# Snoworday/instance-segmentation-attention

Measured on AMD Instinct MI355X. Metric: images/sec @256x256 bs=16 per GPU, higher is better.
Workload: dtype bf16; 1 GPU; train.py step fwd+bwd+update 256x256 bs=16/GPU (bf16); global_batch=16, parallelism=dp1, launch=hipGraph replay

## Files before the change

### instance-segmentation-attention_amd/csrc/conv_fused_bwd.hip

```cpp
#include "common.hpp"
#include "tr_lds.hpp"

int wgrad_slab_reduce_launch(float* ws, float* dw, float* dbias, int gx, int tn, int tk, int N, int cin, int taps,
                             isa_slab_arena* sa, hipStream_t s);

namespace {

struct PwParams {
    const bf16_t *g, *y, *x; bf16_t* dx; const float* w; float* dw;
    int N, K, ldg, ldy, ldx, lddx; long M;
    const float *ysc, *ysh, *ymu, *yis, *yred; float ycnt_inv; int yact; float *ydgamma, *ydbeta;
    const float *xsc, *xsh, *xmu, *xis; int xact; float* xred;
    int accumulate; float* ws;
    const bf16_t* addend; int lda;
    int G;
};

template <int TN, int TK, int YACT, int XMODE>
__global__ __launch_bounds__(256) __attribute__((amdgpu_waves_per_eu(2, 2))) void pw_bn_bwd_kernel(PwParams p) {
    extern __shared__ __attribute__((aligned(16))) char ldsb[];
    constexpr int PMB = 32;
    constexpr int SN = TrStride<TN * 32>::bytes, SK = TrStride<TK * 32>::bytes;
    constexpr int SLAB = PMB * (SN + SK);
    constexpr int VN = TN * 4, VK = TK * 4;
    constexpr int LOADS_N = PMB * VN / 64, LOADS_K = PMB * VK / 64;
    constexpr int RPN = 64 / VN, RPK = 64 / VK;
    constexpr int XACT = XMODE == 1 ? ISA_ACT_RELU6 : (XMODE == 0 ? ISA_ACT_NONE : ACT_RT);
    constexpr int NS = TN * 2;
    const int tid = threadIdx.x, wave = tid >> 6, lane = tid & 63;
    const int r = lane & 31, hh = lane >> 5;
    char* sD = ldsb + wave * SLAB;
    char* sX = sD + PMB * SN;
    const GroupSel gs = group_sel(p.G);
    if (gs.g) {
        const long gm = (long)gs.g * p.M;
        p.g += gm * p.ldg; p.y += gm * p.ldy; p.x += gm * p.ldx; p.dx += gm * p.lddx;
        if (p.addend) p.addend += gm * p.lda;
        p.ysc += gs.g * p.N; p.ysh += gs.g * p.N; p.ymu += gs.g * p.N; p.yis += gs.g * p.N; p.yred += gs.g * ISA_STAT_R * 2 * p.N;
        p.xsc = goff(p.xsc, (long)gs.g * p.K); p.xsh = goff(p.xsh, (long)gs.g * p.K); p.xmu = goff(p.xmu, (long)gs.g * p.K);
        p.xis = goff(p.xis, (long)gs.g * p.K); p.xred = goff(p.xred, (long)gs.g * ISA_STAT_R * 2 * p.K);
    }
    const bool want_xred = XMODE == 1 || (XMODE == 2 && p.xred != nullptr);

    const int cgn = lane % VN, rown = lane / VN, cgk = lane % VK, rowk = lane / VK;
    const int cn0 = cgn * 8, ck0 = cgk * 8;
    const bool nok = cn0 < p.N, kok = ck0 < p.K;
    float* cst = reinterpret_cast<float*>(ldsb + 4 * SLAB);
    float* wl = reinterpret_cast<float*>(ldsb);
    for (int i = tid; i < p.N * p.K; i += 256) wl[i] = p.w[i];
    if (tid < 64) {
        const int cn = min(tid, p.N - 1), ck = min(tid, p.K - 1);
        cst[0 * 64 + tid] = p.ysc[cn]; cst[1 * 64 + tid] = p.ysh[cn]; cst[2 * 64 + tid] = p.ymu[cn];
        float r0 = 0.f, r1 = 0.f;
#pragma unroll
        for (int r = 0; r < ISA_STAT_R; ++r) { r0 += p.yred[r * 2 * p.N + cn]; r1 += p.yred[r * 2 * p.N + p.N + cn]; }
        cst[3 * 64 + tid] = p.yis[cn] * (r1 * p.ycnt_inv);
        cst[4 * 64 + tid] = r0 * p.ycnt_inv;
        if (gs.bx == 0 && tid < p.N) {
            if (p.ydgamma) atomicAdd(p.ydgamma + tid, r1);
            if (p.ydbeta) atomicAdd(p.ydbeta + tid, r0);
        }
        cst[5 * 64 + tid] = (XMODE && p.xsc) ? p.xsc[ck] : 1.f; cst[6 * 64 + tid] = (XMODE && p.xsh) ? p.xsh[ck] : 0.f;
        cst[7 * 64 + tid] = (XMODE && p.xmu) ? p.xmu[ck] : 0.f; cst[8 * 64 + tid] = (XMODE && p.xis) ? p.xis[ck] : 1.f;
    }
    __syncthreads();
    auto ldc = [&](int which, int c0, float (&v)[8]) {
        const f32x4 a = *reinterpret_cast<const f32x4*>(cst + which * 64 + c0), b = *reinterpret_cast<const f32x4*>(cst + which * 64 + c0 + 4);
#pragma unroll
        for (int j = 0; j < 4; ++j) { v[j] = a[j]; v[4 + j] = b[j]; }
    };
    bf16x8 wb[NS][TK];
#pragma unroll
    for (int s = 0; s < NS; ++s)
#pragma unroll
        for (int j = 0; j < TK; ++j)
#pragma unroll
            for (int jj = 0; jj < 8; ++jj) {
                const int n = 16 * s + 8 * hh + jj, k = 32 * j + r;
                wb[s][j][jj] = (bf16_t)((n < p.N && k < p.K) ? wl[n * p.K + k] : 0.f);
            }
    __syncthreads();

    f32x16 acc[TN][TK];
#pragma unroll
    for (int i = 0; i < TN; ++i)
#pragma unroll
        for (int j = 0; j < TK; ++j) acc[i][j] = f32x16{0};
    float s0[8], s1[8];
#pragma unroll
    for (int j = 0; j < 8; ++j) { s0[j] = 0.f; s1[j] = 0.f; }

    bf16x8 rg[LOADS_N], ry[LOADS_N], rx[LOADS_K], rxc[LOADS_K];
    const long nchunks = (p.M + PMB - 1) / PMB;
    auto fetch = [&](long chunk) {
        const long mbase = chunk * PMB;
#pragma unroll
        for (int v = 0; v < LOADS_N; ++v) {
            const long m = mbase + v * RPN + rown;
            rg[v] = bf16x8{0}; ry[v] = bf16x8{0};
            if (m < p.M && nok) {
                rg[v] = *reinterpret_cast<const bf16x8*>(p.g + m * p.ldg + cn0);
                ry[v] = *reinterpret_cast<const bf16x8*>(p.y + m * p.ldy + cn0);
            }
        }
#pragma unroll
        for (int v = 0; v < LOADS_K; ++v) {
            const long m = mbase + v * RPK + rowk;
            rx[v] = bf16x8{0};
            if (m < p.M && kok) rx[v] = *reinterpret_cast<const bf16x8*>(p.x + m * p.ldx + ck0);
        }
    };
    auto stash = [&](long chunk) {
        const long mbase = chunk * PMB;
        {
        float ysc[8], ysh[8], ymu[8], yq[8], yk0[8];
        ldc(0, cn0, ysc); ldc(1, cn0, ysh); ldc(2, cn0, ymu); ldc(3, cn0, yq); ldc(4, cn0, yk0);
#pragma unroll
        for (int v = 0; v < LOADS_N; ++v) {
            const bool ok = (mbase + v * RPN + rown) < p.M && nok;
            bf16x8 o;
#pragma unroll
            for (int j = 0; j < 8; ++j) {
                const float yy = (float)ry[v][j];
                const float dz = (float)rg[v][j] * act_grad_t<YACT>(fmaf(yy, ysc[j], ysh[j]), p.yact);
                const float val = ysc[j] * (dz - yk0[j] - (yy - ymu[j]) * yq[j]);
                o[j] = (bf16_t)((ok && cn0 + j < p.N) ? val : 0.f);
            }
            *reinterpret_cast<bf16x8*>(sD + (v * RPN + rown) * SN + cgn * 16) = o;
        }
        }
        float xsc[8], xsh[8];
        ldc(5, ck0, xsc); ldc(6, ck0, xsh);
#pragma unroll
        for (int v = 0; v < LOADS_K; ++v) {
            const bool ok = (mbase + v * RPK + rowk) < p.M && kok;
            bf16x8 o;
#pragma unroll
            for (int j = 0; j < 8; ++j) {
                const float xr = (float)rx[v][j];
                const float z = XMODE ? act_t<XACT>(fmaf(xr, xsc[j], xsh[j]), p.xact) : xr;
                o[j] = (bf16_t)((ok && ck0 + j < p.K) ? z : 0.f);
            }
            *reinterpret_cast<bf16x8*>(sX + (v * RPK + rowk) * SK + cgk * 16) = o;
            rxc[v] = rx[v];
        }
    };

    const long stride = (long)gs.nbx * 4;
    long chunk = (long)gs.bx * 4 + wave;
    if (chunk < nchunks) fetch(chunk);
    for (; chunk < nchunks; chunk += stride) {
        stash(chunk);
        __builtin_amdgcn_fence(__ATOMIC_RELEASE, "wavefront");
        __builtin_amdgcn_wave_barrier();
        if (chunk + stride < nchunks) fetch(chunk + stride);
        constexpr bool EPI_PREFETCH = TK == 1;
        bf16x8 repi_old[EPI_PREFETCH ? LOADS_K : 1], repi_add[EPI_PREFETCH ? LOADS_K : 1];
        if constexpr (EPI_PREFETCH) {
            const long mb = chunk * PMB;
#pragma unroll
            for (int v = 0; v < LOADS_K; ++v) {
                const long m = mb + v * RPK + rowk;
                repi_old[v] = bf16x8{0}; repi_add[v] = bf16x8{0};
                if (m < p.M && kok) {
                    if (p.accumulate) repi_old[v] = *reinterpret_cast<const bf16x8*>(p.dx + m * p.lddx + ck0);
                    if (p.addend) repi_add[v] = *reinterpret_cast<const bf16x8*>(p.addend + m * p.lda + ck0);
                }
            }
        }
#pragma unroll
        for (int s = 0; s < PMB / 16; ++s) {
            bf16x8 a[TN], b[TK];
#pragma unroll
            for (int i = 0; i < TN; ++i) a[i] = tr_frag(sD, SN, 16 * s, i * 32, lane);
#pragma unroll
            for (int j = 0; j < TK; ++j) b[j] = tr_frag(sX, SK, 16 * s, j * 32, lane);
#pragma unroll
            for (int i = 0; i < TN; ++i)
#pragma unroll
                for (int j = 0; j < TK; ++j)
                    acc[i][j] = __builtin_amdgcn_mfma_f32_32x32x16_bf16(a[i], b[j], acc[i][j], 0, 0, 0);
        }
        f32x16 dxa[TK];
#pragma unroll
        for (int j = 0; j < TK; ++j) dxa[j] = f32x16{0};
#pragma unroll
        for (int s = 0; s < NS; ++s) {
            const bf16x8 a = *reinterpret_cast<const bf16x8*>(sD + r * SN + (16 * s + 8 * hh) * 2);
#pragma unroll
            for (int j = 0; j < TK; ++j)
                dxa[j] = __builtin_amdgcn_mfma_f32_32x32x16_bf16(a, wb[s][j], dxa[j], 0, 0, 0);
        }
        __builtin_amdgcn_fence(__ATOMIC_RELEASE, "wavefront");
        __builtin_amdgcn_wave_barrier();
#pragma unroll
        for (int j = 0; j < TK; ++j)
#pragma unroll
            for (int e = 0; e < 16; ++e) {
                const int row = (e & 3) + 8 * (e >> 2) + 4 * hh;
                *reinterpret_cast<bf16_t*>(sX + row * SK + (32 * j + r) * 2) = (bf16_t)dxa[j][e];
            }
        __builtin_amdgcn_fence(__ATOMIC_RELEASE, "wavefront");
        __builtin_amdgcn_wave_barrier();
        const long mbase = chunk * PMB;
        float xsc[8], xsh[8], xmu[8], xis[8];
        if (want_xred) { ldc(5, ck0, xsc); ldc(6, ck0, xsh); ldc(7, ck0, xmu); ldc(8, ck0, xis); }
#pragma unroll
        for (int v = 0; v < LOADS_K; ++v) {
            const long m = mbase + v * RPK + rowk;
            if (m < p.M && kok) {
                bf16x8 o = *reinterpret_cast<const bf16x8*>(sX + (v * RPK + rowk) * SK + cgk * 16);
                bf16_t* dst = p.dx + m * p.lddx + ck0;
                if (p.accumulate) {
                    bf16x8 old;
                    if constexpr (EPI_PREFETCH) old = repi_old[v]; else old = *reinterpret_cast<const bf16x8*>(dst);
#pragma unroll
                    for (int j = 0; j < 8; ++j) o[j] = (bf16_t)((float)o[j] + (float)old[j]);
                }
                if (p.addend) {
                    bf16x8 ad;
                    if constexpr (EPI_PREFETCH) ad = repi_add[v]; else ad = *reinterpret_cast<const bf16x8*>(p.addend + m * p.lda + ck0);
#pragma unroll
                    for (int j = 0; j < 8; ++j) o[j] = (bf16_t)((float)o[j] + (float)ad[j]);
                }
                *reinterpret_cast<bf16x8*>(dst) = o;
                if (want_xred) {
#pragma unroll
                    for (int j = 0; j < 8; ++j) {
                        const float xr = (float)rxc[v][j];
                        const float dz = (float)o[j] * act_grad_t<XACT>(fmaf(xr, xsc[j], xsh[j]), p.xact);
                        s0[j] += dz; s1[j] += dz * ((xr - xmu[j]) * xis[j]);
                    }
                }
            }
        }
        __builtin_amdgcn_fence(__ATOMIC_RELEASE, "wavefront");
        __builtin_amdgcn_wave_barrier();
    }

    __syncthreads();
    float* red = reinterpret_cast<float*>(ldsb);
    constexpr int ACC_FLOATS = TN * TK * 16 * 64;
    for (int w = 0; w < 4; ++w) {
        if (wave == w) {
#pragma unroll
            for (int i = 0; i < TN; ++i)
#pragma unroll
                for (int j = 0; j < TK; ++j)
#pragma unroll
                    for (int e = 0; e < 16; ++e) {
                        float* q = red + ((i * TK + j) * 16 + e) * 64 + lane;
                        *q = (w == 0 ? 0.f : *q) + acc[i][j][e];
                    }
        }
        __syncthreads();
    }
    constexpr int SLABF = TN * TK * 1024 + TN * 32;
    float* slab = p.ws + (long)blockIdx.x * SLABF;
    if (wave == 0) {
#pragma unroll
        for (int e = 0; e < TN * TK * 16; ++e) slab[e * 64 + lane] = red[e * 64 + lane];
        for (int i = lane; i < TN * 32; i += 64) slab[TN * TK * 1024 + i] = 0.f;
    }
    if (want_xred) {
        __syncthreads();
        float* xr = red;
        for (int i = tid; i < 2 * TK * 32; i += 256) xr[i] = 0.f;
        __syncthreads();
#pragma unroll
        for (int j = 0; j < 8; ++j) {
            const float v0 = row_fold<VK>(s0[j]), v1 = row_fold<VK>(s1[j]);
            if ((lane & 15) < VK) { atomicAdd(&xr[ck0 + j], v0); atomicAdd(&xr[TK * 32 + ck0 + j], v1); }
        }
        __syncthreads();
        for (int i = tid; i < 2 * TK * 32; i += 256) {
            const int which = i / (TK * 32), c = i - which * TK * 32;
            if (c < p.K && xr[i] != 0.f)
                atomicAdd(p.xred + (blockIdx.x & (ISA_STAT_R - 1)) * 2 * p.K + which * p.K + c, xr[i]);
        }
    }
}

template <int TN, int TK, int YACT, int XMODE>
int launch_inst(PwParams& p, long ws_floats, isa_slab_arena* sa, const isa_pro* xfin, int xfin_groups, hipStream_t s) {
    constexpr int SN = TrStride<TN * 32>::bytes, SK = TrStride<TK * 32>::bytes;
    constexpr size_t slab = (size_t)32 * (SN + SK) * 4 + 9 * 64 * 4;
    constexpr size_t redb = ((size_t)TN * TK * 16 * 64 + TN * 32) * 4;
    constexpr size_t lds = slab > redb ? slab : redb;
    const long nchunks = (p.M + 31) / 32;
    const long slabf = (long)TN * TK * 1024 + TN * 32;
    long gx = (nchunks + 3) / 4 * p.G;
    if (gx > 256 * 2) gx = 256 * 2;
    if (int rc = defer_ws(sa, &p.ws, &ws_floats)) return rc;
    const long ws_cap = ws_floats / slabf;
    if (ws_cap < p.G) return sa ? ISA_ENOMEM : ISA_EINVAL;
    if (gx > ws_cap) gx = ws_cap;
    gx = group_grid(gx, p.G);
    if (int rc = fin_standalone(xfin, p.K, xfin_groups, s)) return rc;
    hipLaunchKernelGGL((pw_bn_bwd_kernel<TN, TK, YACT, XMODE>), dim3((unsigned)gx), dim3(256), lds, s, p);
    if (launch_status() != ISA_OK) return ISA_ELAUNCH;
    return wgrad_slab_reduce_launch(p.ws, p.dw, nullptr, (int)gx, TN, TK, p.N, p.K, 1, sa, s);
}

template <int TN, int TK>
int launch_tile(PwParams& p, int xmode, long ws_floats, isa_slab_arena* sa, const isa_pro* xfin, int xfin_groups, hipStream_t s) {
    const bool y6 = p.yact == ISA_ACT_RELU6, y0 = p.yact == ISA_ACT_NONE;
#define PW_X(YA) (xmode == 0 ? launch_inst<TN, TK, YA, 0>(p, ws_floats, sa, xfin, xfin_groups, s) \
                : xmode == 1 ? launch_inst<TN, TK, YA, 1>(p, ws_floats, sa, xfin, xfin_groups, s) \
                             : launch_inst<TN, TK, YA, 2>(p, ws_floats, sa, xfin, xfin_groups, s))
    if (y6) return PW_X(ISA_ACT_RELU6);
    if (y0) return PW_X(ISA_ACT_NONE);
    return PW_X(ACT_RT);
#undef PW_X
}

}

extern "C" int isa_conv1x1_bn_backward(const isa_tensor* g, const isa_tensor* y, const isa_bn_bwd* ybn,
                                       const isa_tensor* x, const isa_pro* xpro, const isa_bn_bwd* xbn,
                                       const float* w, float* dw, const isa_tensor* dx, int32_t accumulate,
                                       const isa_tensor* addend, float* ws, int64_t ws_floats, isa_slab_arena* defer,
                                       void* stream) {
    if (!tensor_ok(g, 8) || !tensor_ok(y, 8) || !tensor_ok(x, 8) || !tensor_ok(dx, 8)) return ISA_EINVAL;
    if (!fin_valid(xpro)) return ISA_EINVAL;
    if (g->dtype != ISA_BF16 || y->dtype != ISA_BF16 || x->dtype != ISA_BF16 || dx->dtype != ISA_BF16) return ISA_EINVAL;
    if (!ybn || !ybn->scale || !ybn->shift || !ybn->mean || !ybn->invstd || !ybn->red || !(ybn->count > 0)) return ISA_EINVAL;
    if (!w || !dw || (!ws && !defer)) return ISA_EINVAL;
    const int N = g->c, K = x->c;
    if (N > 64 || K > 64 || N % 8 || K % 8) return ISA_EINVAL;
    if (y->c != N || dx->c != K) return ISA_EINVAL;
    const isa_tensor* ts[3] = {y, x, dx};
    for (const isa_tensor* t : ts)
        if (t->n != g->n || t->h != g->h || t->w != g->w) return ISA_EINVAL;
    const ProDev xp = make_pro(xpro);
    if (xp.bscale) return ISA_EINVAL;
    if (xbn && (!xbn->mean || !xbn->invstd || !xbn->out_red)) return ISA_EINVAL;
    PwParams p{};
    p.g = (const bf16_t*)g->data; p.y = (const bf16_t*)y->data; p.x = (const bf16_t*)x->data; p.dx = (bf16_t*)dx->data;
    p.w = w; p.dw = dw; p.N = N; p.K = K; p.ldg = g->ld; p.ldy = y->ld; p.ldx = x->ld; p.lddx = dx->ld;
// ... 23 lines not shown
```

### instance-segmentation-attention_amd/csrc/conv_wgrad.hip

```cpp
#include <vector>
#include "common.hpp"
#include "tr_lds.hpp"

int conv3x3_wgrad_tiled_launch(const isa_tensor* x, const isa_tensor* dy, float* dw, float* dbias, float* ws, long ws_floats,
                               isa_slab_arena* sa,
                               hipStream_t s);

namespace {

constexpr int PM = 16;

struct WgParams {
    const void* x; int xh, xw, cin, ldx;
    const void* dy; int dh, dw_, ldd;
    int mh, mw; long M;
    ProDev pro;
    float* dw; float* dbias;
    const int32_t* kmap; int ksrc;
    int N, taps, in_mode, out_mode;
    int groups_k;
    long nchunks;
    long ws_floats;
    int G;
    isa_slab_arena* sa;
// ... 258 lines not shown
        fold_depthwise(d.ws, d.gx, d.gy, d.tk, d.N, d.ksrc, d.dw, d.dbias, lb % d.gy, lb / d.gy, d.rsplit);
    }
}

constexpr long DEFER_MIN_FLOATS = 16L << 20;

static int launch_reduce(const WgParams& p, int gx, int gy, int tn, int tk, hipStream_t s) {
    const int slabf = tn * tk * 1024 + tn * 32;
    const long base_blocks = (long)cdiv(slabf, 256) * gy * p.taps;
    int rsplit = (int)((512 + base_blocks - 1) / base_blocks);
    if (rsplit > 64) rsplit = 64;
    if (rsplit > gx) rsplit = gx;
    if (rsplit < 1) rsplit = 1;
    if (p.sa && p.sa->from_arena) {
        FoldDesc d{p.ws, p.dw, p.dbias, p.kmap, 0, gx, gy, p.taps, p.groups_k, tn, tk, p.N, p.cin, p.ksrc, p.out_mode, 0, 0, 0};
        if (defer_push(p.sa, d, (long)gx * gy * p.taps * slabf)) return ISA_OK;
    }
    WgReduce q{p.ws, p.dw, p.dbias, p.kmap, gx, gy, p.taps, p.groups_k, tn, tk, p.N, p.cin, p.ksrc, p.out_mode, rsplit};
    dim3 grid(cdiv(slabf, 256), gy, p.taps * rsplit);
    hipLaunchKernelGGL(wgrad_reduce_kernel, grid, dim3(256), 0, s, q);
    return launch_status();
}

template <int TN, int TK, int ACT>
__global__ __launch_bounds__(256) void conv_wgrad_bf16_kernel(WgParams p) {
    extern __shared__ __attribute__((aligned(16))) char ldsb[];
    constexpr int PMB = 32;
    constexpr int SN = TrStride<TN * 32>::bytes, SK = TrStride<TK * 32>::bytes;
    constexpr int SLAB = PMB * (SN + SK);
    constexpr int VN = TN * 4, VK = TK * 4;
    constexpr int LOADS_N = PMB * VN / 64, LOADS_K = PMB * VK / 64;
    const int tid = threadIdx.x, wave = tid >> 6, lane = tid & 63;
    const int r = lane & 31, hh = lane >> 5;
    const int gn = blockIdx.y / p.groups_k, gk = blockIdx.y % p.groups_k;
    const int tap = blockIdx.z;
    const int n0 = gn * TN * 32, k0 = gk * TK * 32;
    char* sD = ldsb + wave * SLAB;
    char* sX = sD + PMB * SN;
    const GroupSel gs = group_sel(p.G);
    if (gs.g) {
        p.x = reinterpret_cast<const bf16_t*>(p.x) + (long)gs.g * p.M * p.ldx;
        p.dy = reinterpret_cast<const bf16_t*>(p.dy) + (long)gs.g * p.M * p.ldd;
        p.pro.scale = goff(p.pro.scale, (long)gs.g * p.cin); p.pro.shift = goff(p.pro.shift, (long)gs.g * p.cin);
        p.pro.bscale = goff(p.pro.bscale, (long)gs.g * (p.M / ((long)p.mh * p.mw)) * p.cin);
    }
    const bf16_t* xin = reinterpret_cast<const bf16_t*>(p.x);
    const bf16_t* din = reinterpret_cast<const bf16_t*>(p.dy);
    const bool plain = p.in_mode == ISA_IN_1X1 && p.out_mode == ISA_OUT_PLAIN;

    f32x16 acc[TN][TK];
#pragma unroll
    for (int i = 0; i < TN; ++i)
#pragma unroll
        for (int j = 0; j < TK; ++j) acc[i][j] = f32x16{0};
    float dbs[TN];
#pragma unroll
    for (int i = 0; i < TN; ++i) dbs[i] = 0.f;
    bf16x8 rd[LOADS_N], rx[LOADS_K];
    const long nchunks = (p.M + PMB - 1) / PMB;
    const int cgn = lane % VN, rown = lane / VN, cgk = lane % VK, rowk = lane / VK;
    constexpr int RPN = 64 / VN, RPK = 64 / VK;
    const int cn0 = n0 + cgn * 8, ck0 = k0 + cgk * 8;
    const bool has_aff = p.pro.scale || p.pro.shift;
    const bool has_pro = has_aff || p.pro.bscale || p.pro.act != ISA_ACT_NONE;
    float psc[8], psh[8];
#pragma unroll
    for (int j = 0; j < 8; ++j) {
        const int c = min(ck0 + j, p.cin - 1);
        psc[j] = p.pro.scale ? p.pro.scale[c] : 1.f;
        psh[j] = p.pro.shift ? p.pro.shift[c] : 0.f;
    }

    auto fetch = [&](long chunk) {
        const long mbase = chunk * PMB;
#pragma unroll
        for (int v = 0; v < LOADS_N; ++v) {
            const long m = mbase + v * RPN + rown;
            rd[v] = bf16x8{0};
            if (m < p.M && cn0 < p.N) {
                long row = m;
                if (p.out_mode == ISA_OUT_SHUFFLE2) {
                    const unsigned mu = (unsigned)m, q = mu / (unsigned)p.mw;
                    const int px = (int)(mu - q * (unsigned)p.mw);
                    const unsigned pb = q / (unsigned)p.mh; const int py = (int)(q - pb * (unsigned)p.mh);
                    row = ((long)pb * p.dh + 2 * py + (tap >> 1)) * p.dw_ + 2 * px + (tap & 1);
                }
                const bf16_t* src = din + row * p.ldd + cn0;
                if (cn0 + 8 <= p.N) rd[v] = *reinterpret_cast<const bf16x8*>(src);
                else {
#pragma unroll
                    for (int j = 0; j < 8; ++j) rd[v][j] = (cn0 + j < p.N) ? src[j] : (bf16_t)0.f;
                }
            }
        }
#pragma unroll
        for (int v = 0; v < LOADS_K; ++v) {
            const long m = mbase + v * RPK + rowk;
            rx[v] = bf16x8{0};
            if (m < p.M && ck0 < p.cin) {
                long row = m; bool ok = true; long pb = 0;
                if (!plain || p.pro.bscale) {
                    const unsigned mu = (unsigned)m, q = mu / (unsigned)p.mw;
                    const int px = (int)(mu - q * (unsigned)p.mw);
                    pb = q / (unsigned)p.mh; const int py = (int)(q - (unsigned)pb * (unsigned)p.mh);
                    if (p.in_mode == ISA_IN_3X3) {
                        const int sy = py + tap / 3 - 1, sx = px + tap % 3 - 1;
                        ok = sy >= 0 && sy < p.xh && sx >= 0 && sx < p.xw;
                        row = (pb * p.xh + sy) * p.xw + sx;
                    }
                }
                if (ok) {
                    const bf16_t* src = xin + row * p.ldx + ck0;
                    bf16x8 raw;
                    if (ck0 + 8 <= p.cin) raw = *reinterpret_cast<const bf16x8*>(src);
                    else {
#pragma unroll
                        for (int j = 0; j < 8; ++j) raw[j] = (ck0 + j < p.cin) ? src[j] : (bf16_t)0.f;
                    }
                    if (has_pro) {
                        float z[8];
#pragma unroll
                        for (int j = 0; j < 8; ++j) z[j] = act_t<ACT>(fmaf((float)raw[j], psc[j], psh[j]), p.pro.act);
                        if (p.pro.bscale) {
#pragma unroll
                            for (int j = 0; j < 8; ++j) z[j] *= p.pro.bscale[pb * p.cin + min(ck0 + j, p.cin - 1)];
                        }
                        if (ck0 + 8 > p.cin) {
#pragma unroll
                            for (int j = 0; j < 8; ++j) if (ck0 + j >= p.cin) z[j] = 0.f;
                        }
#pragma unroll
                        for (int j = 0; j < 8; ++j) raw[j] = (bf16_t)z[j];
                    }
                    rx[v] = raw;
                }
            }
        }
    };
    auto stash = [&]() {
#pragma unroll
        for (int v = 0; v < LOADS_N; ++v)
            *reinterpret_cast<bf16x8*>(sD + (v * RPN + rown) * SN + cgn * 16) = rd[v];
#pragma unroll
        for (int v = 0; v < LOADS_K; ++v)
            *reinterpret_cast<bf16x8*>(sX + (v * RPK + rowk) * SK + cgk * 16) = rx[v];
    };

    const long stride = (long)gs.nbx * 4;
    long chunk = (long)gs.bx * 4 + wave;
    if (chunk < nchunks) fetch(chunk);
    for (; chunk < nchunks; chunk += stride) {
        stash();
        __builtin_amdgcn_fence(__ATOMIC_RELEASE, "wavefront");
        __builtin_amdgcn_wave_barrier();
        if (chunk + stride < nchunks) fetch(chunk + stride);
#pragma unroll
        for (int s = 0; s < PMB / 16; ++s) {
            bf16x8 a[TN], b[TK];
#pragma unroll
            for (int i = 0; i < TN; ++i) {
                a[i] = tr_frag(sD, SN, 16 * s, i * 32, lane);
#pragma unroll
                for (int j = 0; j < 8; ++j) dbs[i] += (float)a[i][j];
            }
#pragma unroll
            for (int j = 0; j < TK; ++j) b[j] = tr_frag(sX, SK, 16 * s, j * 32, lane);
#pragma unroll
            for (int i = 0; i < TN; ++i)
#pragma unroll
                for (int j = 0; j < TK; ++j)
                    acc[i][j] = __builtin_amdgcn_mfma_f32_32x32x16_bf16(a[i], b[j], acc[i][j], 0, 0, 0);
        }
        __builtin_amdgcn_fence(__ATOMIC_RELEASE, "wavefront");
        __builtin_amdgcn_wave_barrier();
    }

    __syncthreads();
    float* red = reinterpret_cast<float*>(ldsb);
    constexpr int ACC_FLOATS = TN * TK * 16 * 64;
    for (int w = 0; w < 4; ++w) {
        if (wave == w) {
#pragma unroll
            for (int i = 0; i < TN; ++i)
#pragma unroll
                for (int j = 0; j < TK; ++j)
#pragma unroll
                    for (int e = 0; e < 16; ++e) {
                        float* q = red + ((i * TK + j) * 16 + e) * 64 + lane;
                        *q = (w == 0 ? 0.f : *q) + acc[i][j][e];
                    }
#pragma unroll
            for (int i = 0; i < TN; ++i) {
                const float sv = dbs[i] + __shfl_xor(dbs[i], 32, 64);
                if (hh == 0) { float* q = red + ACC_FLOATS + i * 32 + r; *q = (w == 0 ? 0.f : *q) + sv; }
            }
        }
        __syncthreads();
    }
    if (wave != 0) return;
    constexpr int SLABF = TN * TK * 1024 + TN * 32;
    float* slab = p.ws + (((long)blockIdx.x * gridDim.y + blockIdx.y) * gridDim.z + blockIdx.z) * SLABF;
#pragma unroll
    for (int e = 0; e < TN * TK * 16; ++e) slab[e * 64 + lane] = red[e * 64 + lane];
    for (int i = lane; i < TN * 32; i += 64) slab[TN * TK * 1024 + i] = red[ACC_FLOATS + i];
}

template <int TN, int TK>
int launch_wg_bf16(WgParams& p, int groups_n, const isa_pro* fin, hipStream_t s) {
    constexpr int SN = TrStride<TN * 32>::bytes, SK = TrStride<TK * 32>::bytes;
    const size_t slab = (size_t)32 * (SN + SK) * 4;
    const size_t redb = ((size_t)TN * TK * 16 * 64 + TN * 32) * 4;
    const size_t lds = slab > redb ? slab : redb;
    const int gy = groups_n * p.groups_k;
    const long nchunks = (p.M + 31) / 32;
    const long slabf = (long)TN * TK * 1024 + TN * 32;
    long want = (nchunks + 3) / 4 * p.G;
    long cap = (256L * 2) / ((long)gy * p.taps);
    if (int rc = defer_ws(p.sa, &p.ws, &p.ws_floats)) return rc;
    const long ws_cap = p.ws_floats / (slabf * gy * p.taps);
    if (ws_cap < p.G) return p.sa ? ISA_ENOMEM : ISA_EINVAL;
    if (cap > ws_cap) cap = ws_cap;
    if (cap < 1) cap = 1;
    const int gx = (int)group_grid(want < cap ? want : cap, p.G);
    dim3 grid(gx, gy, p.taps);
    if (int rc = fin_standalone(fin, p.cin, p.G, s)) return rc;
    if (p.pro.act == ISA_ACT_RELU6) hipLaunchKernelGGL((conv_wgrad_bf16_kernel<TN, TK, ISA_ACT_RELU6>), grid, dim3(256), lds, s, p);
    else if (p.pro.act == ISA_ACT_LEAKY && TN == 1 && TK == 1) hipLaunchKernelGGL((conv_wgrad_bf16_kernel<TN, TK, ISA_ACT_LEAKY>), grid, dim3(256), lds, s, p);
    else if (p.pro.act == ISA_ACT_NONE) hipLaunchKernelGGL((conv_wgrad_bf16_kernel<TN, TK, ISA_ACT_NONE>), grid, dim3(256), lds, s, p);
    else hipLaunchKernelGGL((conv_wgrad_bf16_kernel<TN, TK, ACT_RT>), grid, dim3(256), lds, s, p);
    if (launch_status() != ISA_OK) return ISA_ELAUNCH;
    return launch_reduce(p, gx, gy, TN, TK, s);
}


// ... 31 lines not shown
    else { tn = 2; tk = 2; }
    const int groups_n = (nt + tn - 1) / tn;
    p.groups_k = (kt + tk - 1) / tk;
    if constexpr (sizeof(T) == 2) {
        if (tn == 1 && tk == 1) return launch_wg_bf16<1, 1>(p, groups_n, fin, s);
        if (tn == 1 && tk == 2) return launch_wg_bf16<1, 2>(p, groups_n, fin, s);
        if (tn == 2 && tk == 1) return launch_wg_bf16<2, 1>(p, groups_n, fin, s);
        if (tn == 2 && tk == 2) return launch_wg_bf16<2, 2>(p, groups_n, fin, s);
        if (tn == 1 && tk == 4) return launch_wg_bf16<1, 4>(p, groups_n, fin, s);
        if (tn == 4 && tk == 1) return launch_wg_bf16<4, 1>(p, groups_n, fin, s);
        return ISA_EINVAL;
    }
    if (tn == 1 && tk == 1) return launch_wg<T, 1, 1>(p, groups_n, fin, s);
    if (tn == 1 && tk == 2) return launch_wg<T, 1, 2>(p, groups_n, fin, s);
    if (tn == 2 && tk == 1) return launch_wg<T, 2, 1>(p, groups_n, fin, s);
    if (tn == 2 && tk == 2) return launch_wg<T, 2, 2>(p, groups_n, fin, s);
    if (tn == 1 && tk == 4) return launch_wg<T, 1, 4>(p, groups_n, fin, s);
    if (tn == 4 && tk == 1) return launch_wg<T, 4, 1>(p, groups_n, fin, s);
    return ISA_EINVAL;
}

}

extern "C" int isa_conv_wgrad(const isa_tensor* x, const isa_pro* pro, const isa_tensor* dy,
                              float* dw, float* dbias, int32_t in_mode, int32_t out_mode,
                              const int32_t* kmap, int32_t ksrc, float* ws, int64_t ws_floats,
                              isa_slab_arena* defer, void* stream) {
    if (!tensor_ok(x, 8) || !tensor_ok(dy, 8) || !dw || x->dtype != dy->dtype || (!ws && !defer)) return ISA_EINVAL;
    if (!fin_valid(pro)) return ISA_EINVAL;
    if (in_mode == ISA_IN_GATHER2) return ISA_EINVAL;
    WgParams p{};
    p.x = x->data; p.xh = x->h; p.xw = x->w; p.cin = x->c; p.ldx = x->ld;
    p.dy = dy->data; p.dh = dy->h; p.dw_ = dy->w; p.ldd = dy->ld;
    p.mh = x->h; p.mw = x->w; p.M = (long)x->n * x->h * x->w;
    p.pro = make_pro(pro); p.dw = dw; p.dbias = dbias; p.kmap = kmap; p.ksrc = ksrc > 0 ? ksrc : x->c;
    p.in_mode = in_mode; p.out_mode = out_mode; p.ws = ws; p.ws_floats = ws_floats; p.sa = defer;
    if (out_mode == ISA_OUT_SHUFFLE2) {
        if (in_mode != ISA_IN_1X1 || dy->h != 2 * x->h || dy->w != 2 * x->w || dy->n != x->n) return ISA_EINVAL;
        p.taps = 4; p.N = dy->c;
    } else {
        if (dy->h != x->h || dy->w != x->w || dy->n != x->n) return ISA_EINVAL;
        p.taps = in_mode == ISA_IN_3X3 ? 9 : 1; p.N = dy->c;
    }
    p.G = 1;
    const int G = tensor_groups(x);
    if (G > 1 && (p.pro.scale || p.pro.shift)) {
// ... 80 lines not shown
```

### instance-segmentation-attention_amd/csrc/tr_lds.hpp

```cpp
#pragma once
#include "common.hpp"

typedef short s16x4 __attribute__((ext_vector_type(4)));
typedef short s16x8 __attribute__((ext_vector_type(8)));
#define LDS_S16X4(ptr) ((__attribute__((address_space(3))) s16x4*)(ptr))

template <int CH> struct TrStride { static constexpr int bytes = (CH * 2) % 128 == 0 ? CH * 2 + 64 : CH * 2; };

__device__ __forceinline__ bf16x8 tr_frag(const char* tile, int stride_bytes, int pix0, int chan0, int lane) {
    const int g = lane >> 4, i = lane & 15, q = i >> 2, pp = i & 3;
    const char* a = tile + (pix0 + 8 * (g >> 1) + q) * stride_bytes + (chan0 + 16 * (g & 1) + 4 * pp) * 2;
    const s16x4 lo = __builtin_amdgcn_ds_read_tr16_b64_v4i16(LDS_S16X4(a));
    const s16x4 hi = __builtin_amdgcn_ds_read_tr16_b64_v4i16(LDS_S16X4(a + 4 * stride_bytes));
    const s16x8 v = __builtin_shufflevector(lo, hi, 0, 1, 2, 3, 4, 5, 6, 7);
    return __builtin_bit_cast(bf16x8, v);
}
```

Measured before the change: 693.4 images/s.

## Restructure pointwise BN-backward and wgrad kernels: early prefetch, parallel fold, branchless loads

Both backward kernels now issue the first chunk's global loads before the weight and constant setup, so that load latency overlaps with that setup. Guarded loads become branchless loads at clamped addresses, with validity kept as bitmasks or zeroing applied in the stash step. The serialized four-wave LDS accumulation, which needed a block barrier per wave, is replaced by each wave parking its accumulators in its own region and then a parallel 4-way sum on store. In the pointwise kernel the weights are staged as transposed bf16 in LDS so each lane reads them with one vector load. An EPI template flag drops the accumulate/addend epilogue when it is unused, and the x-stat atomics become a slot sum. Optional phase-timing macros are added but compile away by default. The parallel fold uses more LDS, which may reduce occupancy.

```diff
diff --git a/instance-segmentation-attention_amd/csrc/conv_fused_bwd.hip b/instance-segmentation-attention_amd/csrc/conv_fused_bwd.hip
--- a/instance-segmentation-attention_amd/csrc/conv_fused_bwd.hip
+++ b/instance-segmentation-attention_amd/csrc/conv_fused_bwd.hip
@@ -16,9 +16,14 @@
     int G;
 };
 
-template <int TN, int TK, int YACT, int XMODE>
+#ifdef ISA_PHASE_TRACE
+__device__ unsigned long long phase_buf[10];
+#endif
+
+template <int TN, int TK, int YACT, int XMODE, bool EPI>
 __global__ __launch_bounds__(256) __attribute__((amdgpu_waves_per_eu(2, 2))) void pw_bn_bwd_kernel(PwParams p) {
     extern __shared__ __attribute__((aligned(16))) char ldsb[];
+    PHASE_DECL(); PHASE(0);
     constexpr int PMB = 32;
     constexpr int SN = TrStride<TN * 32>::bytes, SK = TrStride<TK * 32>::bytes;
     constexpr int SLAB = PMB * (SN + SK);
@@ -45,9 +50,37 @@
     const int cgn = lane % VN, rown = lane / VN, cgk = lane % VK, rowk = lane / VK;
     const int cn0 = cgn * 8, ck0 = cgk * 8;
     const bool nok = cn0 < p.N, kok = ck0 < p.K;
+    const int cnl = nok ? cn0 : 0, ckl = kok ? ck0 : 0;
+
+    bf16x8 rg[LOADS_N], ry[LOADS_N], rx[LOADS_K], rxc[LOADS_K];
+    const long nchunks = (p.M + PMB - 1) / PMB;
+    auto fetch = [&](long chunk) {
+        const long mbase = chunk * PMB;
+#pragma unroll
+        for (int v = 0; v < LOADS_N; ++v) {
+            const long m = min(mbase + v * RPN + rown, p.M - 1);
+            rg[v] = *reinterpret_cast<const bf16x8*>(p.g + m * p.ldg + cnl);
+            ry[v] = *reinterpret_cast<const bf16x8*>(p.y + m * p.ldy + cnl);
+        }
+#pragma unroll
+        for (int v = 0; v < LOADS_K; ++v) {
+            const long m = min(mbase + v * RPK + rowk, p.M - 1);
+            rx[v] = *reinterpret_cast<const bf16x8*>(p.x + m * p.ldx + ckl);
+        }
+    };
+    const long stride = (long)gs.nbx * 4;
+    long chunk = (long)gs.bx * 4 + wave;
+    if (chunk < nchunks) fetch(chunk);
+
     float* cst = reinterpret_cast<float*>(ldsb + 4 * SLAB);
-    float* wl = reinterpret_cast<float*>(ldsb);
-    for (int i = tid; i < p.N * p.K; i += 256) wl[i] = p.w[i];
+    constexpr int WP = TN * 32 + 8;
+    bf16_t* wl = reinterpret_cast<bf16_t*>(ldsb);
+    float wv[TN * TK * 4];
+#pragma unroll
+    for (int it = 0; it < TN * TK * 4; ++it) {
+        const int i = it * 256 + tid, n = i / (TK * 32), k = i % (TK * 32);
+        wv[it] = p.w[min(n, p.N - 1) * p.K + min(k, p.K - 1)];
+    }
     if (tid < 64) {
         const int cn = min(tid, p.N - 1), ck = min(tid, p.K - 1);
         cst[0 * 64 + tid] = p.ysc[cn]; cst[1 * 64 + tid] = p.ysh[cn]; cst[2 * 64 + tid] = p.ymu[cn];
@@ -63,7 +96,13 @@
         cst[5 * 64 + tid] = (XMODE && p.xsc) ? p.xsc[ck] : 1.f; cst[6 * 64 + tid] = (XMODE && p.xsh) ? p.xsh[ck] : 0.f;
         cst[7 * 64 + tid] = (XMODE && p.xmu) ? p.xmu[ck] : 0.f; cst[8 * 64 + tid] = (XMODE && p.xis) ? p.xis[ck] : 1.f;
     }
+#pragma unroll
+    for (int it = 0; it < TN * TK * 4; ++it) {
+        const int i = it * 256 + tid, n = i / (TK * 32), k = i % (TK * 32);
+        wl[k * WP + n] = (bf16_t)((n < p.N && k < p.K) ? wv[it] : 0.f);
+    }
     __syncthreads();
+    PHASE(1);
     auto ldc = [&](int which, int c0, float (&v)[8]) {
         const f32x4 a = *reinterpret_cast<const f32x4*>(cst + which * 64 + c0), b = *reinterpret_cast<const f32x4*>(cst + which * 64 + c0 + 4);
 #pragma unroll
@@ -74,12 +113,9 @@
     for (int s = 0; s < NS; ++s)
 #pragma unroll
         for (int j = 0; j < TK; ++j)
-#pragma unroll
-            for (int jj = 0; jj < 8; ++jj) {
-                const int n = 16 * s + 8 * hh + jj, k = 32 * j + r;
-                wb[s][j][jj] = (bf16_t)((n < p.N && k < p.K) ? wl[n * p.K + k] : 0.f);
-            }
+            wb[s][j] = *reinterpret_cast<const bf16x8*>(wl + (32 * j + r) * WP + 16 * s + 8 * hh);
     __syncthreads();
+    PHASE(2);
 
     f32x16 acc[TN][TK];
 #pragma unroll
@@ -90,26 +126,6 @@
 #pragma unroll
     for (int j = 0; j < 8; ++j) { s0[j] = 0.f; s1[j] = 0.f; }
 
-    bf16x8 rg[LOADS_N], ry[LOADS_N], rx[LOADS_K], rxc[LOADS_K];
-    const long nchunks = (p.M + PMB - 1) / PMB;
-    auto fetch = [&](long chunk) {
-        const long mbase = chunk * PMB;
-#pragma unroll
-        for (int v = 0; v < LOADS_N; ++v) {
-            const long m = mbase + v * RPN + rown;
-            rg[v] = bf16x8{0}; ry[v] = bf16x8{0};
-            if (m < p.M && nok) {
-                rg[v] = *reinterpret_cast<const bf16x8*>(p.g + m * p.ldg + cn0);
-                ry[v] = *reinterpret_cast<const bf16x8*>(p.y + m * p.ldy + cn0);
-            }
-        }
-#pragma unroll
-        for (int v = 0; v < LOADS_K; ++v) {
-            const long m = mbase + v * RPK + rowk;
-            rx[v] = bf16x8{0};
-            if (m < p.M && kok) rx[v] = *reinterpret_cast<const bf16x8*>(p.x + m * p.ldx + ck0);
-        }
-    };
     auto stash = [&](long chunk) {
         const long mbase = chunk * PMB;
         {
@@ -146,28 +162,24 @@
         }
     };
 
-    const long stride = (long)gs.nbx * 4;
-    long chunk = (long)gs.bx * 4 + wave;
-    if (chunk < nchunks) fetch(chunk);
     for (; chunk < nchunks; chunk += stride) {
         stash(chunk);
         __builtin_amdgcn_fence(__ATOMIC_RELEASE, "wavefront");
         __builtin_amdgcn_wave_barrier();
-        if (chunk + stride < nchunks) fetch(chunk + stride);
-        constexpr bool EPI_PREFETCH = TK == 1;
+        PHASE_ONCE(3);
+        constexpr bool EPI_PREFETCH = EPI && TK == 1;
         bf16x8 repi_old[EPI_PREFETCH ? LOADS_K : 1], repi_add[EPI_PREFETCH ? LOADS_K : 1];
         if constexpr (EPI_PREFETCH) {
             const long mb = chunk * PMB;
 #pragma unroll
             for (int v = 0; v < LOADS_K; ++v) {
-                const long m = mb + v * RPK + rowk;
+                const long m = min(mb + v * RPK + rowk, p.M - 1);
                 repi_old[v] = bf16x8{0}; repi_add[v] = bf16x8{0};
-                if (m < p.M && kok) {
-                    if (p.accumulate) repi_old[v] = *reinterpret_cast<const bf16x8*>(p.dx + m * p.lddx + ck0);
-                    if (p.addend) repi_add[v] = *reinterpret_cast<const bf16x8*>(p.addend + m * p.lda + ck0);
-                }
-            }
-        }
+                if (p.accumulate) repi_old[v] = *reinterpret_cast<const bf16x8*>(p.dx + m * p.lddx + ckl);
+                if (p.addend) repi_add[v] = *reinterpret_cast<const bf16x8*>(p.addend + m * p.lda + ckl);
+            }
+        }
+        if (chunk + stride < nchunks) fetch(chunk + stride);
 #pragma unroll
         for (int s = 0; s < PMB / 16; ++s) {
             bf16x8 a[TN], b[TK];
@@ -211,17 +223,19 @@
             if (m < p.M && kok) {
                 bf16x8 o = *reinterpret_cast<const bf16x8*>(sX + (v * RPK + rowk) * SK + cgk * 16);
                 bf16_t* dst = p.dx + m * p.lddx + ck0;
-                if (p.accumulate) {
-                    bf16x8 old;
-                    if constexpr (EPI_PREFETCH) old = repi_old[v]; else old = *reinterpret_cast<const bf16x8*>(dst);
-#pragma unroll
-                    for (int j = 0; j < 8; ++j) o[j] = (bf16_t)((float)o[j] + (float)old[j]);
-                }
-                if (p.addend) {
-                    bf16x8 ad;
-                    if constexpr (EPI_PREFETCH) ad = repi_add[v]; else ad = *reinterpret_cast<const bf16x8*>(p.addend + m * p.lda + ck0);
-#pragma unroll
-                    for (int j = 0; j < 8; ++j) o[j] = (bf16_t)((float)o[j] + (float)ad[j]);
+                if constexpr (EPI) {
+                    if (p.accumulate) {
+                        bf16x8 old;
+                        if constexpr (EPI_PREFETCH) old = repi_old[v]; else old = *reinterpret_cast<const bf16x8*>(dst);
+#pragma unroll
+                        for (int j = 0; j < 8; ++j) o[j] = (bf16_t)((float)o[j] + (float)old[j]);
+                    }
+                    if (p.addend) {
+                        bf16x8 ad;
+                        if constexpr (EPI_PREFETCH) ad = repi_add[v]; else ad = *reinterpret_cast<const bf16x8*>(p.addend + m * p.lda + ck0);
+#pragma unroll
+                        for (int j = 0; j < 8; ++j) o[j] = (bf16_t)((float)o[j] + (float)ad[j]);
+                    }
                 }
                 *reinterpret_cast<bf16x8*>(dst) = o;
                 if (want_xred) {
@@ -238,54 +252,44 @@
         __builtin_amdgcn_wave_barrier();
     }
 
+    PHASE(4);
     __syncthreads();
-    float* red = reinterpret_cast<float*>(ldsb);
-    constexpr int ACC_FLOATS = TN * TK * 16 * 64;
-    for (int w = 0; w < 4; ++w) {
-        if (wave == w) {
-#pragma unroll
-            for (int i = 0; i < TN; ++i)
-#pragma unroll
-                for (int j = 0; j < TK; ++j)
-#pragma unroll
-                    for (int e = 0; e < 16; ++e) {
-                        float* q = red + ((i * TK + j) * 16 + e) * 64 + lane;
-                        *q = (w == 0 ? 0.f : *q) + acc[i][j][e];
-                    }
-        }
-        __syncthreads();
-    }
+    PHASE(5);
+    float* part = reinterpret_cast<float*>(ldsb);
+    float* xs = part + fold_part_floats<TN, TK>();
+    fold_park<TN, TK>(part, acc, wave, lane);
+    if (want_xred) {
+        float* slot = xs + (wave * 4 + (lane >> 4)) * (2 * TK * 32);
+#pragma unroll
+        for (int j = 0; j < 8; ++j) {
+            const float v0 = row_fold<VK>(s0[j]), v1 = row_fold<VK>(s1[j]);
+            if ((lane & 15) < VK) { slot[ck0 + j] = v0; slot[TK * 32 + ck0 + j] = v1; }
+        }
+    }
+    __syncthreads();
+    PHASE(6);
     constexpr int SLABF = TN * TK * 1024 + TN * 32;
     float* slab = p.ws + (long)blockIdx.x * SLABF;
-    if (wave == 0) {
-#pragma unroll
-        for (int e = 0; e < TN * TK * 16; ++e) slab[e * 64 + lane] = red[e * 64 + lane];
-        for (int i = lane; i < TN * 32; i += 64) slab[TN * TK * 1024 + i] = 0.f;
-    }
-    if (want_xred) {
-        __syncthreads();
-        float* xr = red;
-        for (int i = tid; i < 2 * TK * 32; i += 256) xr[i] = 0.f;
-        __syncthreads();
-#pragma unroll
-        for (int j = 0; j < 8; ++j) {
-            const float v0 = row_fold<VK>(s0[j]), v1 = row_fold<VK>(s1[j]);
-            if ((lane & 15) < VK) { atomicAdd(&xr[ck0 + j], v0); atomicAdd(&xr[TK * 32 + ck0 + j], v1); }
-        }
-        __syncthreads();
-        for (int i = tid; i < 2 * TK * 32; i += 256) {
-            const int which = i / (TK * 32), c = i - which * TK * 32;
-            if (c < p.K && xr[i] != 0.f)
-                atomicAdd(p.xred + (blockIdx.x & (ISA_STAT_R - 1)) * 2 * p.K + which * p.K + c, xr[i]);
-        }
-    }
+    fold_store<TN, TK>(part, slab, tid);
+    PHASE(7);
+    if (tid < TN * 32) slab[TN * TK * 1024 + tid] = 0.f;
+    if (want_xred && tid < 2 * TK * 32) {
+        float v = 0.f;
+#pragma unroll
+        for (int sl = 0; sl < 16; ++sl) v += xs[sl * (2 * TK * 32) + tid];
+        const int which = tid / (TK * 32), c = tid - which * TK * 32;
+        if (c < p.K && v != 0.f)
+            atomicAdd(p.xred + (blockIdx.x & (ISA_STAT_R - 1)) * 2 * p.K + which * p.K + c, v);
+    }
+    PHASE(8);
+    PHASE_FLUSH(phase_buf);
 }
 
 template <int TN, int TK, int YACT, int XMODE>
 int launch_inst(PwParams& p, long ws_floats, isa_slab_arena* sa, const isa_pro* xfin, int xfin_groups, hipStream_t s) {
     constexpr int SN = TrStride<TN * 32>::bytes, SK = TrStride<TK * 32>::bytes;
     constexpr size_t slab = (size_t)32 * (SN + SK) * 4 + 9 * 64 * 4;
-    constexpr size_t redb = ((size_t)TN * TK * 16 * 64 + TN * 32) * 4;
+    constexpr size_t redb = ((size_t)fold_part_floats<TN, TK>() + 16 * 2 * TK * 32) * 4;
     constexpr size_t lds = slab > redb ? slab : redb;
     const long nchunks = (p.M + 31) / 32;
     const long slabf = (long)TN * TK * 1024 + TN * 32;
@@ -297,7 +301,8 @@
     if (gx > ws_cap) gx = ws_cap;
     gx = group_grid(gx, p.G);
     if (int rc = fin_standalone(xfin, p.K, xfin_groups, s)) return rc;
-    hipLaunchKernelGGL((pw_bn_bwd_kernel<TN, TK, YACT, XMODE>), dim3((unsigned)gx), dim3(256), lds, s, p);
+    if (p.accumulate || p.addend) hipLaunchKernelGGL((pw_bn_bwd_kernel<TN, TK, YACT, XMODE, true>), dim3((unsigned)gx), dim3(256), lds, s, p);
+    else hipLaunchKernelGGL((pw_bn_bwd_kernel<TN, TK, YACT, XMODE, false>), dim3((unsigned)gx), dim3(256), lds, s, p);
     if (launch_status() != ISA_OK) return ISA_ELAUNCH;
     return wgrad_slab_reduce_launch(p.ws, p.dw, nullptr, (int)gx, TN, TK, p.N, p.K, 1, sa, s);
 }
@@ -315,6 +320,10 @@
 }
 
 }
+
+#ifdef ISA_PHASE_TRACE
+extern "C" int isa_phase_trace_pw(unsigned long long* out) { return hipMemcpyFromSymbol(out, HIP_SYMBOL(phase_buf), sizeof(phase_buf)) == hipSuccess ? ISA_OK : ISA_ELAUNCH; }
+#endif
 
 extern "C" int isa_conv1x1_bn_backward(const isa_tensor* g, const isa_tensor* y, const isa_bn_bwd* ybn,
                                        const isa_tensor* x, const isa_pro* xpro, const isa_bn_bwd* xbn,
diff --git a/instance-segmentation-attention_amd/csrc/conv_wgrad.hip b/instance-segmentation-attention_amd/csrc/conv_wgrad.hip
--- a/instance-segmentation-attention_amd/csrc/conv_wgrad.hip
+++ b/instance-segmentation-attention_amd/csrc/conv_wgrad.hip
@@ -304,9 +304,14 @@
     return launch_status();
 }
 
+#ifdef ISA_PHASE_TRACE
+__device__ unsigned long long phase_buf[10];
+#endif
+
 template <int TN, int TK, int ACT>
 __global__ __launch_bounds__(256) void conv_wgrad_bf16_kernel(WgParams p) {
     extern __shared__ __attribute__((aligned(16))) char ldsb[];
+    PHASE_DECL(); PHASE(0);
     constexpr int PMB = 32;
     constexpr int SN = TrStride<TN * 32>::bytes, SK = TrStride<TK * 32>::bytes;
     constexpr int SLAB = PMB * (SN + SK);
@@ -345,6 +350,54 @@
     const int cn0 = n0 + cgn * 8, ck0 = k0 + cgk * 8;
     const bool has_aff = p.pro.scale || p.pro.shift;
     const bool has_pro = has_aff || p.pro.bscale || p.pro.act != ISA_ACT_NONE;
+    const bool nok = cn0 < p.N, kok = ck0 < p.cin;
+    const int cnl = nok ? cn0 : 0, ckl = kok ? ck0 : 0;
+    const bool xdiv = !plain || p.pro.bscale;
+
+    unsigned okd = 0, okx = 0;
+    int pbv[LOADS_K];
+#pragma unroll
+    for (int v = 0; v < LOADS_K; ++v) pbv[v] = 0;
+    auto fetch = [&](long chunk) {
+        const long mbase = chunk * PMB;
+        okd = 0; okx = 0;
+#pragma unroll
+        for (int v = 0; v < LOADS_N; ++v) {
+            const long m = mbase + v * RPN + rown;
+            if (m < p.M && nok) okd |= 1u << v;
+            long row = m < p.M ? m : p.M - 1;
+            if (p.out_mode == ISA_OUT_SHUFFLE2) {
+                const unsigned mu = (unsigned)row, q = mu / (unsigned)p.mw;
+                const int px = (int)(mu - q * (unsigned)p.mw);
+                const unsigned pb = q / (unsigned)p.mh; const int py = (int)(q - pb * (unsigned)p.mh);
+                row = ((long)pb * p.dh + 2 * py + (tap >> 1)) * p.dw_ + 2 * px + (tap & 1);
+            }
+            rd[v] = *reinterpret_cast<const bf16x8*>(din + row * p.ldd + cnl);
+        }
+#pragma unroll
+        for (int v = 0; v < LOADS_K; ++v) {
+            const long m = mbase + v * RPK + rowk;
+            long row = m < p.M ? m : p.M - 1;
+            bool ok = m < p.M && kok;
+            if (xdiv) {
+                const unsigned mu = (unsigned)row, q = mu / (unsigned)p.mw;
+                const int px = (int)(mu - q * (unsigned)p.mw);
+                const long pb = q / (unsigned)p.mh; const int py = (int)(q - (unsigned)pb * (unsigned)p.mh);
+                pbv[v] = (int)pb;
+                if (p.in_mode == ISA_IN_3X3) {
+                    const int sy = py + tap / 3 - 1, sx = px + tap % 3 - 1;
+                    ok = ok && sy >= 0 && sy < p.xh && sx >= 0 && sx < p.xw;
+                    row = (pb * p.xh + min(max(sy, 0), p.xh - 1)) * p.xw + min(max(sx, 0), p.xw - 1);
+                }
+            }
+            if (ok) okx |= 1u << v;
+            rx[v] = *reinterpret_cast<const bf16x8*>(xin + row * p.ldx + ckl);
+        }
+    };
+
+    const long stride = (long)gs.nbx * 4;
+    long chunk = (long)gs.bx * 4 + wave;
+    if (chunk < nchunks) fetch(chunk);
     float psc[8], psh[8];
 #pragma unroll
     for (int j = 0; j < 8; ++j) {
@@ -352,89 +405,57 @@
         psc[j] = p.pro.scale ? p.pro.scale[c] : 1.f;
         psh[j] = p.pro.shift ? p.pro.shift[c] : 0.f;
     }
-
-    auto fetch = [&](long chunk) {
-        const long mbase = chunk * PMB;
+    float bsr[8];
+    int bsi = -1;
+#pragma unroll
+    for (int j = 0; j < 8; ++j) bsr[j] = 1.f;
+
+    auto stash = [&]() {
 #pragma unroll
         for (int v = 0; v < LOADS_N; ++v) {
-            const long m = mbase + v * RPN + rown;
-            rd[v] = bf16x8{0};
-            if (m < p.M && cn0 < p.N) {
-                long row = m;
-                if (p.out_mode == ISA_OUT_SHUFFLE2) {
-                    const unsigned mu = (unsigned)m, q = mu / (unsigned)p.mw;
-                    const int px = (int)(mu - q * (unsigned)p.mw);
-                    const unsigned pb = q / (unsigned)p.mh; const int py = (int)(q - pb * (unsigned)p.mh);
-                    row = ((long)pb * p.dh + 2 * py + (tap >> 1)) * p.dw_ + 2 * px + (tap & 1);
+            bf16x8 o = rd[v];
+            if (!((okd >> v) & 1)) o = bf16x8{0};
+            else if (cn0 + 8 > p.N) {
+#pragma unroll
+                for (int j = 0; j < 8; ++j) if (cn0 + j >= p.N) o[j] = (bf16_t)0.f;
+            }
+            *reinterpret_cast<bf16x8*>(sD + (v * RPN + rown) * SN + cgn * 16) = o;
+        }
+#pragma unroll
+        for (int v = 0; v < LOADS_K; ++v) {
+            bf16x8 raw = rx[v];
+            const bool ok = (okx >> v) & 1;
+            if (has_pro) {
+                float z[8];
+#pragma unroll
+                for (int j = 0; j < 8; ++j) z[j] = act_t<ACT>(fmaf((float)raw[j], psc[j], psh[j]), p.pro.act);
+                if (p.pro.bscale) {
+                    if (ok && pbv[v] != bsi) {
+                        bsi = pbv[v];
+#pragma unroll
+                        for (int j = 0; j < 8; ++j) bsr[j] = p.pro.bscale[(long)bsi * p.cin + min(ck0 + j, p.cin - 1)];
+                    }
+#pragma unroll
+                    for (int j = 0; j < 8; ++j) z[j] *= bsr[j];
                 }
-                const bf16_t* src = din + row * p.ldd + cn0;
-                if (cn0 + 8 <= p.N) rd[v] = *reinterpret_cast<const bf16x8*>(src);
-                else {
-#pragma unroll
-                    for (int j = 0; j < 8; ++j) rd[v][j] = (cn0 + j < p.N) ? src[j] : (bf16_t)0.f;
-                }
-            }
-        }
-#pragma unroll
-        for (int v = 0; v < LOADS_K; ++v) {
-            const long m = mbase + v * RPK + rowk;
-            rx[v] = bf16x8{0};
-            if (m < p.M && ck0 < p.cin) {
-                long row = m; bool ok = true; long pb = 0;
-                if (!plain || p.pro.bscale) {
-                    const unsigned mu = (unsigned)m, q = mu / (unsigned)p.mw;
-                    const int px = (int)(mu - q * (unsigned)p.mw);
-                    pb = q / (unsigned)p.mh; const int py = (int)(q - (unsigned)pb * (unsigned)p.mh);
-                    if (p.in_mode == ISA_IN_3X3) {
-                        const int sy = py + tap / 3 - 1, sx = px + tap % 3 - 1;
-                        ok = sy >= 0 && sy < p.xh && sx >= 0 && sx < p.xw;
-                        row = (pb * p.xh + sy) * p.xw + sx;
-                    }
-                }
-                if (ok) {
-                    const bf16_t* src = xin + row * p.ldx + ck0;
-                    bf16x8 raw;
-                    if (ck0 + 8 <= p.cin) raw = *reinterpret_cast<const bf16x8*>(src);
-                    else {
-#pragma unroll
-                        for (int j = 0; j < 8; ++j) raw[j] = (ck0 + j < p.cin) ? src[j] : (bf16_t)0.f;
-                    }
-                    if (has_pro) {
-                        float z[8];
-#pragma unroll
-                        for (int j = 0; j < 8; ++j) z[j] = act_t<ACT>(fmaf((float)raw[j], psc[j], psh[j]), p.pro.act);
-                        if (p.pro.bscale) {
-#pragma unroll
-                            for (int j = 0; j < 8; ++j) z[j] *= p.pro.bscale[pb * p.cin + min(ck0 + j, p.cin - 1)];
-                        }
-                        if (ck0 + 8 > p.cin) {
-#pragma unroll
-                            for (int j = 0; j < 8; ++j) if (ck0 + j >= p.cin) z[j] = 0.f;
-                        }
-#pragma unroll
-                        for (int j = 0; j < 8; ++j) raw[j] = (bf16_t)z[j];
-                    }
-                    rx[v] = raw;
-                }
-            }
+#pragma unroll
+                for (int j = 0; j < 8; ++j) raw[j] = (bf16_t)z[j];
+            }
+            if (!ok) raw = bf16x8{0};
+            else if (ck0 + 8 > p.cin) {
+#pragma unroll
+                for (int j = 0; j < 8; ++j) if (ck0 + j >= p.cin) raw[j] = (bf16_t)0.f;
+            }
+            *reinterpret_cast<bf16x8*>(sX + (v * RPK + rowk) * SK + cgk * 16) = raw;
         }
     };
-    auto stash = [&]() {
-#pragma unroll
-        for (int v = 0; v < LOADS_N; ++v)
-            *reinterpret_cast<bf16x8*>(sD + (v * RPN + rown) * SN + cgn * 16) = rd[v];
-#pragma unroll
-        for (int v = 0; v < LOADS_K; ++v)
-            *reinterpret_cast<bf16x8*>(sX + (v * RPK + rowk) * SK + cgk * 16) = rx[v];
-    };
-
-    const long stride = (long)gs.nbx * 4;
-    long chunk = (long)gs.bx * 4 + wave;
-    if (chunk < nchunks) fetch(chunk);
+
+    PHASE(1);
     for (; chunk < nchunks; chunk += stride) {
         stash();
         __builtin_amdgcn_fence(__ATOMIC_RELEASE, "wavefront");
         __builtin_amdgcn_wave_barrier();
+        PHASE_ONCE(3);
         if (chunk + stride < nchunks) fetch(chunk + stride);
 #pragma unroll
         for (int s = 0; s < PMB / 16; ++s) {
@@ -457,41 +478,33 @@
         __builtin_amdgcn_wave_barrier();
     }
 
+    PHASE(4);
     __syncthreads();
-    float* red = reinterpret_cast<float*>(ldsb);
-    constexpr int ACC_FLOATS = TN * TK * 16 * 64;
-    for (int w = 0; w < 4; ++w) {
-        if (wave == w) {
-#pragma unroll
-            for (int i = 0; i < TN; ++i)
-#pragma unroll
-                for (int j = 0; j < TK; ++j)
-#pragma unroll
-                    for (int e = 0; e < 16; ++e) {
-                        float* q = red + ((i * TK + j) * 16 + e) * 64 + lane;
-                        *q = (w == 0 ? 0.f : *q) + acc[i][j][e];
-                    }
-#pragma unroll
-            for (int i = 0; i < TN; ++i) {
-                const float sv = dbs[i] + __shfl_xor(dbs[i], 32, 64);
-                if (hh == 0) { float* q = red + ACC_FLOATS + i * 32 + r; *q = (w == 0 ? 0.f : *q) + sv; }
-            }
-        }
-        __syncthreads();
-    }
-    if (wave != 0) return;
+    PHASE(5);
+    float* part = reinterpret_cast<float*>(ldsb);
+    float* dbp = part + fold_part_floats<TN, TK>();
+    fold_park<TN, TK>(part, acc, wave, lane);
+#pragma unroll
+    for (int i = 0; i < TN; ++i) {
+        const float sv = dbs[i] + __shfl_xor(dbs[i], 32, 64);
+        if (hh == 0) dbp[wave * TN * 32 + i * 32 + r] = sv;
+    }
+    __syncthreads();
+    PHASE(6);
     constexpr int SLABF = TN * TK * 1024 + TN * 32;
     float* slab = p.ws + (((long)blockIdx.x * gridDim.y + blockIdx.y) * gridDim.z + blockIdx.z) * SLABF;
-#pragma unroll
-    for (int e = 0; e < TN * TK * 16; ++e) slab[e * 64 + lane] = red[e * 64 + lane];
-    for (int i = lane; i < TN * 32; i += 64) slab[TN * TK * 1024 + i] = red[ACC_FLOATS + i];
+    fold_store<TN, TK>(part, slab, tid);
+    if (tid < TN * 32)
+        slab[TN * TK * 1024 + tid] = 0.f + dbp[tid] + dbp[TN * 32 + tid] + dbp[2 * TN * 32 + tid] + dbp[3 * TN * 32 + tid];
+    PHASE(7);
+    PHASE_FLUSH(phase_buf);
 }
 
 template <int TN, int TK>
 int launch_wg_bf16(WgParams& p, int groups_n, const isa_pro* fin, hipStream_t s) {
     constexpr int SN = TrStride<TN * 32>::bytes, SK = TrStride<TK * 32>::bytes;
     const size_t slab = (size_t)32 * (SN + SK) * 4;
-    const size_t redb = ((size_t)TN * TK * 16 * 64 + TN * 32) * 4;
+    const size_t redb = ((size_t)fold_part_floats<TN, TK>() + 4 * TN * 32) * 4;
     const size_t lds = slab > redb ? slab : redb;
     const int gy = groups_n * p.groups_k;
     const long nchunks = (p.M + 31) / 32;
@@ -569,6 +582,10 @@
 
 }
 
+#ifdef ISA_PHASE_TRACE
+extern "C" int isa_phase_trace_wg(unsigned long long* out) { return hipMemcpyFromSymbol(out, HIP_SYMBOL(phase_buf), sizeof(phase_buf)) == hipSuccess ? ISA_OK : ISA_ELAUNCH; }
+#endif
+
 extern "C" int isa_conv_wgrad(const isa_tensor* x, const isa_pro* pro, const isa_tensor* dy,
                               float* dw, float* dbias, int32_t in_mode, int32_t out_mode,
                               const int32_t* kmap, int32_t ksrc, float* ws, int64_t ws_floats,
diff --git a/instance-segmentation-attention_amd/csrc/tr_lds.hpp b/instance-segmentation-attention_amd/csrc/tr_lds.hpp
--- a/instance-segmentation-attention_amd/csrc/tr_lds.hpp
+++ b/instance-segmentation-attention_amd/csrc/tr_lds.hpp
@@ -7,6 +7,39 @@
 
 template <int CH> struct TrStride { static constexpr int bytes = (CH * 2) % 128 == 0 ? CH * 2 + 64 : CH * 2; };
 
+#ifdef ISA_PHASE_TRACE
+#define PHASE_DECL() unsigned long long ph_[10] = {0, 0, 0, 0, 0, 0, 0, 0, 0, 0}
+#define PHASE(i) (ph_[i] = wall_clock64())
+#define PHASE_ONCE(i) do { if (ph_[i] == 0) ph_[i] = wall_clock64(); } while (0)
+#define PHASE_FLUSH(buf) do { if (blockIdx.x + blockIdx.y + blockIdx.z == 0 && threadIdx.x == 0) { _Pragma("unroll") for (int i_ = 0; i_ < 10; ++i_) (buf)[i_] = ph_[i_]; } } while (0)
+#else
+#define PHASE_DECL() do {} while (0)
+#define PHASE(i) do {} while (0)
+#define PHASE_ONCE(i) do {} while (0)
+#define PHASE_FLUSH(buf) do {} while (0)
+#endif
+
+template <int TN, int TK> constexpr int fold_part_floats() { return 4 * TN * TK * 1024; }
+template <int TN, int TK>
+__device__ __forceinline__ void fold_park(float* part, const f32x16 (&acc)[TN][TK], int wave, int lane) {
+    float* mine = part + wave * (TN * TK * 1024) + lane;
+#pragma unroll
+    for (int i = 0; i < TN; ++i)
+#pragma unroll
+        for (int j = 0; j < TK; ++j)
+#pragma unroll
+            for (int e = 0; e < 16; ++e) mine[((i * TK + j) * 16 + e) * 64] = acc[i][j][e];
+}
+template <int TN, int TK>
+__device__ __forceinline__ void fold_store(const float* part, float* slab, int tid) {
+    constexpr int ACC = TN * TK * 1024;
+#pragma unroll
+    for (int i = 0; i < ACC / 256; ++i) {
+        const float* q = part + i * 256 + tid;
+        slab[i * 256 + tid] = 0.f + q[0] + q[ACC] + q[2 * ACC] + q[3 * ACC];
+    }
+}
+
 __device__ __forceinline__ bf16x8 tr_frag(const char* tile, int stride_bytes, int pix0, int chan0, int lane) {
     const int g = lane >> 4, i = lane & 15, q = i >> 2, pp = i & 3;
     const char* a = tile + (pix0 + 8 * (g >> 1) + q) * stride_bytes + (chan0 + 16 * (g & 1) + 4 * pp) * 2;
```

Measured after the change: 718.9 images/s (median of 6 runs). 3.7% higher.
